# mx-strk/InformationBottleneckDecodingLDPC

Measured on AMD Instinct MI355X. Metric: decoded codewords/sec + achieved HBM GB/s, DVB-S2 N=64800 i_max=50, higher is better.
Workload: dtype u4

## Files before the change

### informationbottleneckdecodingldpc_amd/csrc/ib_kernels.hip

```cpp
#include <algorithm>
#include <type_traits>

#include "common.h"

namespace ibl {


typedef __attribute__((address_space(3))) const uint8_t lds8_t;
__device__ __forceinline__ uint32_t lu(uint32_t x, uint32_t c) {
  asm("" : "+v"(x));
  return *(lds8_t*)(size_t)(x + c);
}
__device__ __forceinline__ uint32_t luc(uint32_t t, uint32_t q, uint32_t c) {
  uint32_t x;
  static_assert(kRowSh == 12, "luc's shift is the row shift of the table layout");
  asm("v_lshl_or_b32 %0, %1, 12, %2" : "=v"(x) : "v"(t), "v"(q));
  return *(lds8_t*)(size_t)(x + c);
}
typedef __attribute__((address_space(3))) const uint64_t lds64_t;
__device__ __forceinline__ uint64_t colf(uint32_t m, uint32_t cb) {
  uint32_t x;
  asm("v_lshl_or_b32 %0, %1, 8, %2" : "=v"(x) : "v"(m), "v"(cb));
  return *(lds64_t*)(size_t)x;
}
__device__ __forceinline__ uint32_t csel(uint64_t col, uint32_t sh) {
  uint64_t r;
  asm("v_lshrrev_b64 %0, %1, %2" : "=v"(r) : "v"(sh), "v"(col));
  return (uint32_t)r;
}
__device__ __forceinline__ uint32_t lds_base(const uint8_t* p) { return (uint32_t)(size_t)(lds8_t*)p; }
__device__ __forceinline__ void lds_at_zero(const uint8_t* lds) {
  if (lds_base(lds) != 0u) __builtin_trap();
}

__device__ __forceinline__ uint32_t qidx(uint32_t m, uint32_t lane4) { return (m << kColSh) | lane4; }

__device__ __forceinline__ uint32_t valid_mask4(int remaining) {
  return remaining >= 4 ? 0xFu : (remaining <= 0 ? 0u : ((1u << remaining) - 1u));
}

__device__ __forceinline__ bool gate_open(const int32_t* gate, int lane) {
  if (!gate) return true;
  return __ballot(gate[lane] != 0) != 0ull;
}

constexpr int kStageR = 4;
#ifndef IBL_STAGE_UNITS
#define IBL_STAGE_UNITS 0
#endif
__device__ __forceinline__ void stage_tables(uint8_t* lds, const uint32_t* img, int nreg) {
  if constexpr (IBL_STAGE_UNITS) {
    uint4* l4 = reinterpret_cast<uint4*>(lds);
    const int n = (int)(lds_of_quads(nreg) / 16), bd = blockDim.x;
    for (int u = threadIdx.x; u < n; u += 4 * bd) {
      uint32_t w[4];
      bool ok[4];
#pragma unroll
      for (int k = 0; k < 4; ++k) {
        const int v = u + k * bd, q = ((v >> 12) << 1) | ((v >> 3) & 1);
        ok[k] = v < n && q < nreg;
        w[k] = ok[k] ? img[q * 256 + ((v >> 4) & 255)] : 0u;
      }
#pragma unroll
      for (int k = 0; k < 4; ++k)
        if (ok[k]) l4[u + k * bd] = make_uint4(w[k], w[k], w[k], w[k]);
    }
    return;
  }
  const int nraw = nreg * 256, lane = threadIdx.x & 63;
  const int wv = threadIdx.x >> 6, nwv = blockDim.x >> 6, nchunk = (nraw + 63) >> 6;
  for (int c0 = 0; c0 < nchunk; c0 += kStageR * nwv) {
    uint32_t v[kStageR];
#pragma unroll
    for (int k = 0; k < kStageR; ++k) {
      const int r = (c0 + wv + k * nwv) * 64 + lane;
      v[k] = r < nraw ? img[r] : 0u;
    }
#pragma unroll
    for (int k = 0; k < kStageR; ++k) {
      const int c = c0 + wv + k * nwv;
      if (c >= nchunk) break;
#pragma unroll
      for (int p = 0; p < 8; ++p) {
        const int src = 8 * p + (lane >> 3), r = c * 64 + src;
        const uint32_t w = __shfl(v[k], src, 64);
        if (r < nraw)
          *reinterpret_cast<uint4*>(lds + quad_off(r >> 8) + (uint32_t)(r & 255) * 256u + 16u * (uint32_t)(lane & 7)) =
              make_uint4(w, w, w, w);
      }
    }
  }
}

__device__ __forceinline__ void stage_cols(uint8_t* dst, const uint32_t* cimg, int ncs) {
  uint32_t* l32 = reinterpret_cast<uint32_t*>(dst);
  const int n = ncs * 1024;
  for (int i = threadIdx.x; i < n; i += blockDim.x) l32[i] = cimg[((i >> 10) << 5) | (((i >> 6) & 15) << 1) | (i & 1)];
}

__device__ __forceinline__ uint32_t nib(uint32_t w, int k) { return __builtin_amdgcn_ubfe(w, 4 * k, 4); }
__device__ __forceinline__ uint32_t colq(uint32_t w, int k, uint32_t lane4) {
  static_assert(kColSh == 8, "colq places the column in byte 1");
  const uint32_t src = (k & 1) ? ((w >> 4) & 0x0F0F0F0Fu) : (w & 0x0F0F0F0Fu);
  return __builtin_amdgcn_perm(src, lane4, 0x03020000u | ((4u + (uint32_t)(k >> 1)) << 8));
}

__device__ __forceinline__ uint32_t valid_nib8(int remaining) {
  return remaining >= 8 ? 0xFFFFFFFFu : (remaining <= 0 ? 0u : ((1u << (4 * remaining)) - 1u));
}

template <int W> struct RowVec;
template <> struct RowVec<1> { typedef uint32_t T; };
template <> struct RowVec<2> { typedef uint2 T; };
template <> struct RowVec<4> { typedef uint4 T; };

#ifndef IBL_NT_CN
#define IBL_NT_CN 1
#endif
#ifndef IBL_NT
#define IBL_NT 1
#endif
typedef uint32_t u32x2_t __attribute__((ext_vector_type(2)));
typedef uint32_t u32x4_t __attribute__((ext_vector_type(4)));
template <int W> struct RowNV;
template <> struct RowNV<1> { typedef uint32_t T; };
template <> struct RowNV<2> { typedef u32x2_t T; };
template <> struct RowNV<4> { typedef u32x4_t T; };

template <int W, bool NT = false>
__device__ __forceinline__ void load_row(const uint8_t* p, uint32_t (&r)[W]) {
  if constexpr (NT) {
    using T = typename RowNV<W>::T;
    const T v = __builtin_nontemporal_load(reinterpret_cast<const T*>(p));
    if constexpr (W == 1) {
      r[0] = v;
    } else {
#pragma unroll
      for (int i = 0; i < W; ++i) r[i] = v[i];
    }
  } else {
    const auto v = *reinterpret_cast<const typename RowVec<W>::T*>(p);
    if constexpr (W == 1) {
      r[0] = v;
    } else if constexpr (W == 2) {
      r[0] = v.x; r[1] = v.y;
    } else {
      r[0] = v.x; r[1] = v.y; r[2] = v.z; r[3] = v.w;
    }
  }
}

template <int W, bool NT = false>
__device__ __forceinline__ void store_row(uint8_t* p, const uint32_t (&r)[W]) {
  if constexpr (NT) {
    using T = typename RowNV<W>::T;
    T v;
    if constexpr (W == 1) {
      v = r[0];
    } else {
#pragma unroll
      for (int i = 0; i < W; ++i) v[i] = r[i];
    }
    __builtin_nontemporal_store(v, reinterpret_cast<T*>(p));
  } else if constexpr (W == 1) {
    *reinterpret_cast<uint32_t*>(p) = r[0];
  } else if constexpr (W == 2) {
    *reinterpret_cast<uint2*>(p) = make_uint2(r[0], r[1]);
  } else {
    *reinterpret_cast<uint4*>(p) = make_uint4(r[0], r[1], r[2], r[3]);
  }
}


template <int MAXD>
constexpr int rowW() { return MAXD <= 8 ? kW : 1; }
template <int MAXD>
constexpr int chunkOf() { return 512 * rowW<MAXD>(); }
static_assert(kLightD <= 8, "light item buffers must fit the MAXD=8 bodies");

template <int MAXD, int W_ = rowW<MAXD>()>
struct ItemBuf {
  static constexpr int kMax = MAXD, W = W_;
  uint32_t row[MAXD][W];
  uint32_t tgv;
  uint32_t chw[W];
  int d, st, node;
  uint32_t off;
  int cwb;
  int fc, fv0, fv1, fd0, fd1;
};

struct PhaseItems {
  int first, pos0, nch;
};

template <class Buf, bool VN, bool GATHER, int FOLD = 0>
__device__ __forceinline__ void fetch_item(const IbFastArgs& a, int item, int lane, Buf& b, const PhaseItems& pi) {
  constexpr int W = Buf::W, MAXD = Buf::kMax;
  const int rel = item - pi.first;
  const int q = __builtin_amdgcn_readfirstlane(rel / pi.nch);
  const int chunk = __builtin_amdgcn_readfirstlane(rel - q * pi.nch);
  const int pos = pi.pos0 + q;
  const int node = sload(a.info, 4 * pos);
  b.node = node;
  b.st = sload(a.info, 4 * pos + 1);
  b.d = sload(a.info, 4 * pos + 2);
  if constexpr (FOLD != 0) {
    const int32_t* rec = a.fold + (size_t)kIbFoldRec * node;
    b.fc = sload(rec, 0);
    b.fv0 = sload(rec, 1);
    b.fv1 = sload(rec, 2);
    b.fd0 = sload(rec, 3);
    b.fd1 = sload(rec, 4);
  }
  b.off = (uint32_t)(chunk * (256 * W) + lane * 4 * W);
  b.cwb = chunk * (512 * W) + lane * 8 * W;
#pragma unroll
  for (int j = 0; j < MAXD; ++j) {
    const int e = b.st + min(j, b.d - 1);
    const uint8_t* row = GATHER ? a.ch8 + (size_t)sload(a.gather, e) * a.ldb : a.in + (size_t)e * a.ldb;
    load_row<W, VN ? (bool)IBL_NT : ((bool)IBL_NT_CN && !GATHER)>(row + b.off, b.row[j]);
  }
  if (VN) {
    load_row<W, IBL_NT>(a.ch8 + (size_t)node * a.ldb + b.off, b.chw);
  } else {
#pragma unroll
    for (int i = 0; i < W; ++i) b.chw[i] = 0;
  }
  b.tgv = (uint32_t)a.tgt[b.st + min(lane, b.d - 1)];
}

template <bool VN, class Buf>
__device__ __forceinline__ void settle(const Buf& b) {
  constexpr int W = Buf::W;
#pragma unroll
  for (int j = 0; j < Buf::kMax; ++j)
#pragma unroll
    for (int i = 0; i < W; ++i) asm volatile("" ::"v"(b.row[j][i]));
  if constexpr (VN) {
#pragma unroll
    for (int i = 0; i < W; ++i) asm volatile("" ::"v"(b.chw[i]));
  }
  asm volatile("" ::"v"(b.tgv));
}

__device__ __forceinline__ uint32_t pack4n(const uint32_t (&t)[4], int g) {
  return (t[0] | (t[1] << 4) | (t[2] << 8) | (t[3] << 12)) << (16 * g);
}

#ifndef IBL_SCHED_FILE
#define IBL_SCHED_FILE "ib_sched.inc"
#endif
#include IBL_SCHED_FILE

template <int D, int NCW = 8>
__device__ __forceinline__ void cn_word(uint32_t lane4, const uint32_t (&in)[D], uint32_t fbase,
                                        const uint32_t (&cb)[4], uint32_t (&outw)[D]) {
#pragma unroll 1
  for (int k0 = 0; k0 < NCW; k0 += cn_sched_s(D)) cn_group<D>(lane4, in, fbase, cb, outw, k0);
}

template <int D, int FC>
__device__ __forceinline__ void cn_word_fold(uint32_t lane4, const uint32_t (&in)[D], uint32_t fbase,
                                             const uint32_t (&cb)[4], uint32_t lane4c, uint32_t ch0, uint32_t ch1,
                                             uint32_t (&outw)[D]) {
#pragma unroll 1
  for (int k0 = 0; k0 < 8; k0 += cn_sched_s(D)) cn_group_fold<D, FC>(lane4, in, fbase, cb, lane4c, ch0, ch1, outw, k0);
}
__device__ __forceinline__ uint32_t fold_word(uint32_t w, uint32_t ch, uint32_t lane4c) {
  uint32_t r = 0;
#pragma unroll
  for (int g = 0; g < 2; ++g) {
    uint32_t t[4];
#pragma unroll
    for (int s = 0; s < 4; ++s) t[s] = luc(nib(w, 4 * g + s), colq(ch, 4 * g + s, lane4c), 0u);
    r |= pack4n(t, g);
  }
  return r;
}

__device__ __forceinline__ void col_bases(const int8_t (&cc)[4], uint32_t lane8c, uint32_t (&cb)[4]) {
#pragma unroll
  for (int i = 0; i < 4; ++i) cb[i] = lane8c + ((uint32_t)cc[i] << 12);
}

template <int D, bool GATHER, class Buf, int FC = 0, bool KEEP = false>
__device__ __forceinline__ void cn_compute(const IbFastArgs& a, uint32_t lane4, uint32_t lane8c, const Buf& b,
                                           int fslot, bool do_par, bool& unsat, uint8_t* fout = nullptr) {
  constexpr int W = Buf::W;
  uint32_t outw[D][W], trow[D], cb[4];
  uint32_t chf[2][W] = {};
  if constexpr (FC != 0 && !GATHER) {
    if constexpr ((FC & 1) != 0) load_row<W>(a.ch8 + (size_t)b.fv0 * (uint32_t)a.ldb + b.off, chf[0]);
    if constexpr ((FC & 2) != 0) load_row<W>(a.ch8 + (size_t)b.fv1 * (uint32_t)a.ldb + b.off, chf[1]);
  }
  col_bases(a.ccol[D], lane8c, cb);
#pragma unroll
  for (int w = 0; w < D; ++w) trow[w] = __builtin_amdgcn_readlane(b.tgv, w);
  const uint32_t fbase = slot_off(fslot);
  if (do_par) {
    const uint32_t bias = (uint32_t)(8 - a.half) * 0x11111111u;
    uint32_t any = 0;
#pragma unroll
    for (int i = 0; i < W; ++i) {
      uint32_t x = (D & 1) ? 0x88888888u : 0u;
#pragma unroll
      for (int j = 0; j < D; ++j) x ^= b.row[j][i] + bias;
      any |= x & 0x88888888u & valid_nib8(a.B - b.cwb - 8 * i);
    }
    if (__ballot(any != 0) != 0ull) unsat = true;
  }
#pragma unroll
  for (int i = 0; i < W; ++i) {
    uint32_t in[D], o[D];
#pragma unroll
    for (int j = 0; j < D; ++j) {
      in[j] = b.row[j][i];
      o[j] = 0;
    }
    if constexpr (D == 2) {
      if (a.match) {
#pragma unroll
        for (int g = 0; g < 2; ++g) {
          uint32_t t0[4], t1[4];
#pragma unroll
          for (int s = 0; s < 4; ++s) {
            t0[s] = lu((nib(in[1], 4 * g + s) << kRowSh) + lane4, fbase);
            t1[s] = lu((nib(in[0], 4 * g + s) << kRowSh) + lane4, fbase);
          }
          o[0] |= pack4n(t0, g);
          o[1] |= pack4n(t1, g);
        }
      } else {
        o[0] = in[1];
        o[1] = in[0];
      }
    } else if constexpr (FC != 0 && !KEEP) {
      const uint32_t c0 = GATHER ? in[D - 2] : chf[0][i], c1 = GATHER ? in[D - 1] : chf[1][i];
      cn_word_fold<D, FC>(lane4, in, fbase, cb, lane4 + slot_off(a.fold_slot), c0, c1, o);
    } else {
      cn_word<D>(lane4, in, fbase, cb, o);
    }
#pragma unroll
    for (int w = 0; w < D; ++w) outw[w][i] = o[w];
  }
  if constexpr (FC == 0 || KEEP) {
#pragma unroll
    for (int w = 0; w < D; ++w) store_row<W, (bool)IBL_NT_CN>(a.out + (size_t)trow[w] * (uint32_t)a.ldb + b.off, outw[w]);
  }
  if constexpr (FC != 0 && KEEP) {
    const uint32_t lane4c = lane4 + slot_off(a.fold_slot);
#pragma unroll
    for (int fa = 0; fa < 2; ++fa) {
      if (!((FC >> fa) & 1)) continue;
      uint32_t fw[W];
#pragma unroll
      for (int i = 0; i < W; ++i) fw[i] = fold_word(outw[D - 2 + fa][i], GATHER ? b.row[D - 2 + fa][i] : chf[fa][i], lane4c);
      store_row<W, (bool)IBL_NT_CN>(fout + (size_t)(uint32_t)(fa ? b.fd1 : b.fd0) * (uint32_t)a.ldb + b.off, fw);
    }
  } else if constexpr (FC != 0) {
#pragma unroll
    for (int w = 0; w < D - 2; ++w) store_row<W, (bool)IBL_NT_CN>(a.out + (size_t)trow[w] * (uint32_t)a.ldb + b.off, outw[w]);
    if constexpr ((FC & 1) != 0) {
      store_row<W, (bool)IBL_NT_CN>(fout + (size_t)(uint32_t)b.fd0 * (uint32_t)a.ldb + b.off, outw[D - 2]);
    } else {
      store_row<W, (bool)IBL_NT_CN>(a.out + (size_t)trow[D - 2] * (uint32_t)a.ldb + b.off, outw[D - 2]);
    }
    if constexpr ((FC & 2) != 0) {
      store_row<W, (bool)IBL_NT_CN>(fout + (size_t)(uint32_t)b.fd1 * (uint32_t)a.ldb + b.off, outw[D - 1]);
    } else {
      store_row<W, (bool)IBL_NT_CN>(a.out + (size_t)trow[D - 1] * (uint32_t)a.ldb + b.off, outw[D - 1]);
    }
  }
}

template <int D, bool GATHER, bool KEEP, class Buf>
__device__ __forceinline__ void cn_compute_fold(const IbFastArgs& a, uint32_t lane4, uint32_t lane8c, const Buf& b,
                                                int fslot, bool do_par, bool& unsat) {
  if constexpr (D >= 3 && D <= 8) {
    uint8_t* fout = a.fout;
    asm volatile("" : "+s"(fout));
    switch (b.fc) {
      case 1: cn_compute<D, GATHER, Buf, 1, KEEP>(a, lane4, lane8c, b, fslot, do_par, unsat, fout); return;
      case 2: cn_compute<D, GATHER, Buf, 2, KEEP>(a, lane4, lane8c, b, fslot, do_par, unsat, fout); return;
      case 3: cn_compute<D, GATHER, Buf, 3, KEEP>(a, lane4, lane8c, b, fslot, do_par, unsat, fout); return;
      default: break;
    }
  }
  cn_compute<D, GATHER>(a, lane4, lane8c, b, fslot, do_par, unsat);
}

template <int D, int NCW = 8>
__device__ __forceinline__ void vn_word(uint32_t lane4, const uint32_t (&in)[D], uint32_t chw,
                                        uint32_t fbase, const uint32_t (&cb)[4], uint32_t (&outw)[D]) {
#pragma unroll 1
  for (int k0 = 0; k0 < NCW; k0 += vn_sched_s(D)) vn_group<D>(lane4, in, chw, fbase, cb, outw, k0);
}

template <int D, class Buf>
__device__ __forceinline__ void vn_compute(const IbFastArgs& a, uint32_t lane4, uint32_t lane8c, const Buf& b,
                                           int fslot) {
  constexpr int W = Buf::W;
  uint32_t outw[D][W], trow[D], cb[4];
  col_bases(a.ccol[D], lane8c, cb);
#pragma unroll
  for (int w = 0; w < D; ++w) trow[w] = __builtin_amdgcn_readlane(b.tgv, w);
  const uint32_t fbase = slot_off(fslot);
#pragma unroll
  for (int i = 0; i < W; ++i) {
    if constexpr (D == 1) {
      outw[0][i] = b.chw[i];
    } else {
      uint32_t in[D], o[D];
#pragma unroll
      for (int j = 0; j < D; ++j) {
        in[j] = b.row[j][i];
        o[j] = 0;
      }
      vn_word<D>(lane4, in, b.chw[i], fbase, cb, o);
#pragma unroll
      for (int w = 0; w < D; ++w) outw[w][i] = o[w];
    }
  }
#pragma unroll
  for (int w = 0; w < D; ++w) store_row<W, IBL_NT>(a.out + (size_t)trow[w] * (uint32_t)a.ldb + b.off, outw[w]);
}

__device__ __forceinline__ void store4(void* out, int dtype, size_t row_off, int cw0, int B, bool aligned,
                                       uint32_t packed) {
  if (dtype == kU8) {
    uint8_t* p = reinterpret_cast<uint8_t*>(out) + row_off + cw0;
    if (aligned && cw0 + 4 <= B) {
      *reinterpret_cast<uint32_t*>(p) = packed;
    } else {
#pragma unroll
      for (int s = 0; s < 4; ++s)
        if (cw0 + s < B) p[s] = (uint8_t)(packed >> (8 * s));
    }
  } else {
    int32_t* p = reinterpret_cast<int32_t*>(out) + row_off + cw0;
    if (aligned && cw0 + 4 <= B) {
      int4 v = make_int4(packed & 0xff, (packed >> 8) & 0xff, (packed >> 16) & 0xff, packed >> 24);
      *reinterpret_cast<int4*>(p) = v;
    } else {
#pragma unroll
      for (int s = 0; s < 4; ++s)
        if (cw0 + s < B) p[s] = (int32_t)((packed >> (8 * s)) & 0xff);
    }
  }
}

template <int D>
__device__ __forceinline__ void dec_item(const IbDecArgs& a, uint32_t lane4, int node,
                                         int st, uint32_t off, int cwb) {
  uint32_t inw[D];
#pragma unroll
  for (int j = 0; j < D; ++j) inw[j] = *reinterpret_cast<const uint32_t*>(a.vin + (size_t)(st + j) * a.ldb + off);
  const uint32_t cw = *reinterpret_cast<const uint32_t*>(a.ch8 + (size_t)node * a.ldb + off);
#pragma unroll
  for (int g = 0; g < 2; ++g) {
    if (cwb + 4 * g >= a.B) break;
    uint32_t packed = 0;
#pragma unroll
    for (int s = 0; s < 4; ++s) {
      const int k = 4 * g + s;
      uint32_t Q = lu((nib(cw, k) << kRowSh) + qidx(nib(inw[0], k), lane4), 0);
#pragma unroll
      for (int l = 1; l < D; ++l) Q = luc(Q, qidx(nib(inw[l], k), lane4), slot_off(l));
      packed |= Q << (8 * s);
    }
    store4(a.out, a.out_dtype, (size_t)node * a.B, cwb + 4 * g, a.B, a.aligned != 0, packed);
  }
}

#define IBL_DEG_CASES(X) X(2) X(3) X(4) X(5) X(6) X(7) X(8) X(9) X(10) X(11) X(12) X(13) X(14) X(15) X(16)
#define IBL_DEG_CASES8(X) X(2) X(3) X(4) X(5) X(6) X(7) X(8)

__device__ __forceinline__ int* lds_counters(const uint8_t* lds, const IbFastArgs& a) {
  return reinterpret_cast<int*>(const_cast<uint8_t*>(lds) + lds_of_quads(a.nt) + (size_t)a.ncs * kColImg);
// ... 205 lines not shown
#define IBL_WPE8C IBL_WPE8
#endif
template <int MAXD, bool GATHER, int FOLD = 0>
__global__ __launch_bounds__(MAXD <= 8 ? IBL_LB8C : IBL_LB16, MAXD <= 8 ? IBL_WPE8C : 1) void ib_cn_fast(IbFastArgs a) {
  static_assert(FOLD == 0 || MAXD <= 8, "the max-degree-16 bodies do not fold");
  extern __shared__ __attribute__((aligned(16))) uint8_t lds[];
  if (!gate_open(a.gate, threadIdx.x & 63)) return;
  lds_at_zero(lds);
  stage_pass(lds, a);
  __syncthreads();
  ib_pass<MAXD, false, GATHER, FOLD>(a, lds);
}

template <int MAXD>
__global__ __launch_bounds__(MAXD <= 8 ? IBL_LB8 : IBL_LB16, MAXD <= 8 ? IBL_WPE8 : 1) void ib_vn_fast(IbFastArgs a) {
  extern __shared__ __attribute__((aligned(16))) uint8_t lds[];
  if (!gate_open(a.gate, threadIdx.x & 63)) return;
  lds_at_zero(lds);
  stage_pass(lds, a);
  __syncthreads();
  ib_pass<MAXD, true, false>(a, lds);
}

__global__ __launch_bounds__(1024) void ib_dec_fast(IbDecArgs a) {
  extern __shared__ __attribute__((aligned(16))) uint8_t lds[];
  const int lane = threadIdx.x & 63;
  const int L = __builtin_amdgcn_readfirstlane(*a.iters);
  lds_at_zero(lds);
  stage_tables(lds, a.img + (size_t)L * a.nt * 256, a.nt);
  __syncthreads();
  const uint32_t lane4 = (uint32_t)(lane & 31) << 2;
  const int wpb = blockDim.x >> 6;
  const int gw = blockIdx.x * wpb + (threadIdx.x >> 6), nw = gridDim.x * wpb;
  const int nitems = a.n_nodes * a.nchunks;
  for (int item = gw; item < nitems; item += nw) {
    const int node = __builtin_amdgcn_readfirstlane(item / a.nchunks);
    const int chunk = __builtin_amdgcn_readfirstlane(item - node * a.nchunks);
    const int d = a.deg[node], st = a.start[node];
    const uint32_t off = (uint32_t)(chunk * (kChunkDec / 2) + lane * 4);
    const int cwb = chunk * kChunkDec + lane * 8;
    if (cwb >= a.B) continue;
    switch (d) {
      case 1: dec_item<1>(a, lane4, node, st, off, cwb); break;
#define X(D) case D: dec_item<D>(a, lane4, node, st, off, cwb); break;
      IBL_DEG_CASES(X)
#undef X
      default: break;
    }
  }
}

template <int D, bool GATHER>
__device__ __forceinline__ void cn_small_item(const IbFastArgs& a, uint32_t lane4, int st, int c, bool do_par,
                                              bool& unsat) {
  uint32_t in[D], o[D];
  int tg[D];
  const uint32_t off = 4u * (uint32_t)c;
#pragma unroll
  for (int j = 0; j < D; ++j) {
    const int e = st + j;
    const uint8_t* row = GATHER ? a.ch8 + (size_t)a.gather[e] * a.ldb : a.in + (size_t)e * a.ldb;
    in[j] = *reinterpret_cast<const uint32_t*>(row + off);
    tg[j] = a.tgt[e];
    o[j] = 0;
  }
  if (do_par) {
    const uint32_t bias = (uint32_t)(8 - a.half) * 0x11111111u;
    uint32_t x = (D & 1) ? 0x88888888u : 0u;
#pragma unroll
    for (int j = 0; j < D; ++j) x ^= in[j] + bias;
    if (x & 0x88888888u & valid_nib8(a.B - 8 * c)) unsat = true;
  }
  const uint32_t fbase = slot_off(a.fslot[D]);
  if constexpr (D == 2) {
    if (a.match) {
#pragma unroll
      for (int g = 0; g < 2; ++g) {
        uint32_t t0[4], t1[4];
#pragma unroll
        for (int s = 0; s < 4; ++s) {
          t0[s] = lu((nib(in[1], 4 * g + s) << kRowSh) + lane4, fbase);
          t1[s] = lu((nib(in[0], 4 * g + s) << kRowSh) + lane4, fbase);
        }
        o[0] |= pack4n(t0, g);
        o[1] |= pack4n(t1, g);
      }
    } else {
      o[0] = in[1];
      o[1] = in[0];
    }
  } else {
    const uint32_t cb[4] = {0, 0, 0, 0};
    if (a.B - 8 * c <= 4) cn_word<D, 4>(lane4, in, fbase, cb, o);
    else cn_word<D>(lane4, in, fbase, cb, o);
  }
#pragma unroll
  for (int w = 0; w < D; ++w) *reinterpret_cast<uint32_t*>(a.out + (size_t)tg[w] * a.ldb + off) = o[w];
}

template <int D>
__device__ __forceinline__ void vn_small_item(const IbFastArgs& a, uint32_t lane4, int node, int st, int c) {
  uint32_t in[D], o[D];
  int tg[D];
  const uint32_t off = 4u * (uint32_t)c;
#pragma unroll
  for (int j = 0; j < D; ++j) {
    in[j] = *reinterpret_cast<const uint32_t*>(a.in + (size_t)(st + j) * a.ldb + off);
    tg[j] = a.tgt[st + j];
    o[j] = 0;
  }
  const uint32_t chw = *reinterpret_cast<const uint32_t*>(a.ch8 + (size_t)node * a.ldb + off);
  if constexpr (D == 1) {
    o[0] = chw;
  } else {
    const uint32_t cb[4] = {0, 0, 0, 0};
    if (a.B - 8 * c <= 4) vn_word<D, 4>(lane4, in, chw, slot_off(a.fslot[D]), cb, o);
    else vn_word<D>(lane4, in, chw, slot_off(a.fslot[D]), cb, o);
  }
#pragma unroll
  for (int w = 0; w < D; ++w) *reinterpret_cast<uint32_t*>(a.out + (size_t)tg[w] * a.ldb + off) = o[w];
}

#ifndef IBL_SMALL_CONTIG
#define IBL_SMALL_CONTIG 1
#endif
template <bool NODE, class Args, class Body>
__device__ __forceinline__ void small_items(const Args& a, int lane, Body&& body) {
  const int wpb = blockDim.x >> 6;
  const int gw = __builtin_amdgcn_readfirstlane(blockIdx.x * wpb + (threadIdx.x >> 6));
  const int nw = gridDim.x * wpb, nitems = a.n_tasks * a.nwords;
  for (int item = gw; item < nitems; item += nw) {
    const int t = __builtin_amdgcn_readfirstlane(item / a.nwords);
    const int c = __builtin_amdgcn_readfirstlane(item - t * a.nwords);
    const int p0 = sload(a.task, 4 * t), cnt = sload(a.task, 4 * t + 1), d = sload(a.task, 4 * t + 2);
    const int st1 = IBL_SMALL_CONTIG ? sload(a.task, 4 * t + 3) : 0;
    if (lane < cnt) {
      int node = 0, st;
      if (st1 != 0) {
        st = st1 - 1 + lane * d;
        if constexpr (NODE) node = sload(a.info, 4 * p0) + lane;
      } else {
        st = a.info[4 * (p0 + lane) + 1];
        if constexpr (NODE) node = a.info[4 * (p0 + lane)];
      }
      body(node, st, c, d);
    }
  }
}

template <int MAXD, bool GATHER>
__global__ __launch_bounds__(kSmallBlock) void ib_cn_small(IbFastArgs a) {
  extern __shared__ __attribute__((aligned(16))) uint8_t lds[];
  const int lane = threadIdx.x & 63;
  if (!gate_open(a.gate, lane)) return;
  lds_at_zero(lds);
  stage_tables(lds, a.img, a.nt);
  __syncthreads();
  const uint32_t lane4 = (uint32_t)(lane & 31) << 2;
  const bool do_par = !GATHER && a.unsat != nullptr;
  bool unsat = false;
  small_items<false>(a, lane, [&](int, int st, int c, int d) __attribute__((always_inline)) {
    switch (d) {
#define X(D) case D: if constexpr (D <= MAXD) cn_small_item<D, GATHER>(a, lane4, st, c, do_par, unsat); break;
      IBL_DEG_CASES(X)
#undef X
      default: break;
    }
  });
  if (do_par && __ballot(unsat) != 0ull && lane == 0)
    atomicOr(&a.unsat[(blockIdx.x * (blockDim.x >> 6) + (threadIdx.x >> 6)) & (kShards - 1)], 1);
}

template <int MAXD>
__global__ __launch_bounds__(kSmallBlock) void ib_vn_small(IbFastArgs a) {
  extern __shared__ __attribute__((aligned(16))) uint8_t lds[];
  const int lane = threadIdx.x & 63;
  if (!gate_open(a.gate, lane)) return;
  lds_at_zero(lds);
  stage_tables(lds, a.img, a.nt);
  __syncthreads();
  const uint32_t lane4 = (uint32_t)(lane & 31) << 2;
  small_items<true>(a, lane, [&](int node, int st, int c, int d) __attribute__((always_inline)) {
    switch (d) {
      case 1: vn_small_item<1>(a, lane4, node, st, c); break;
#define X(D) case D: if constexpr (D <= MAXD) vn_small_item<D>(a, lane4, node, st, c); break;
      IBL_DEG_CASES(X)
#undef X
      default: break;
    }
  });
}

__global__ __launch_bounds__(kSmallBlock) void ib_dec_small(IbDecArgs a) {
  extern __shared__ __attribute__((aligned(16))) uint8_t lds[];
  const int lane = threadIdx.x & 63;
  const int L = __builtin_amdgcn_readfirstlane(*a.iters);
  lds_at_zero(lds);
  stage_tables(lds, a.img + (size_t)L * a.nt * 256, a.nt);
  __syncthreads();
  const uint32_t lane4 = (uint32_t)(lane & 31) << 2;
  small_items<true>(a, lane, [&](int node, int st, int c, int d) __attribute__((always_inline)) {
    const uint32_t off = 4u * (uint32_t)c;
    switch (d) {
      case 1: dec_item<1>(a, lane4, node, st, off, 8 * c); break;
#define X(D) case D: dec_item<D>(a, lane4, node, st, off, 8 * c); break;
      IBL_DEG_CASES(X)
#undef X
      default: break;
    }
  });
}

#ifndef IBL_FUSED_UNROLL
#define IBL_FUSED_UNROLL 1
#endif
template <int D, int NCW>
__device__ __forceinline__ void fused_cn_word(uint32_t lane4, const uint32_t (&in)[D], uint32_t fbase,
                                              const uint32_t (&cb)[4], uint32_t (&o)[D]) {
  if constexpr (IBL_FUSED_UNROLL && D <= 6) {
#pragma unroll
    for (int k0 = 0; k0 < NCW; k0 += cn_sched_s(D)) cn_group<D>(lane4, in, fbase, cb, o, k0);
  } else {
    cn_word<D, NCW>(lane4, in, fbase, cb, o);
  }
}
template <int D, int NCW>
__device__ __forceinline__ void fused_vn_word(uint32_t lane4, const uint32_t (&in)[D], uint32_t chw, uint32_t fbase,
                                              const uint32_t (&cb)[4], uint32_t (&o)[D]) {
  if constexpr (IBL_FUSED_UNROLL && D <= 4) {
#pragma unroll
    for (int k0 = 0; k0 < NCW; k0 += vn_sched_s(D)) vn_group<D>(lane4, in, chw, fbase, cb, o, k0);
  } else {
    vn_word<D, NCW>(lane4, in, chw, fbase, cb, o);
  }
}

template <int D, int NCW>
__device__ __forceinline__ void fused_cn_dword(uint32_t* msg, int first, int cnt, int lane, uint32_t lane4,
                                               const IbFusedArgs& a, bool do_par, uint32_t vmask, bool& unsat) {
  uint32_t in[D], o[D];
#pragma unroll
  for (int j = 0; j < D; ++j) {
    in[j] = msg[first + j * cnt + lane];
    o[j] = 0;
  }
  if (do_par) {
    const uint32_t bias = (uint32_t)(8 - a.half) * 0x11111111u;
    uint32_t x = (D & 1) ? 0x88888888u : 0u;
#pragma unroll
    for (int j = 0; j < D; ++j) x ^= in[j] + bias;
    if (x & 0x88888888u & vmask) unsat = true;
  }
  const uint32_t fbase = slot_off(a.cn_fslot[D]);
  if constexpr (D == 2) {
    if (a.match) {
#pragma unroll
      for (int g = 0; g < NCW / 4; ++g) {
        uint32_t t0[4], t1[4];
#pragma unroll
        for (int s = 0; s < 4; ++s) {
          t0[s] = lu((nib(in[1], 4 * g + s) << kRowSh) + lane4, fbase);
          t1[s] = lu((nib(in[0], 4 * g + s) << kRowSh) + lane4, fbase);
        }
        o[0] |= pack4n(t0, g);
        o[1] |= pack4n(t1, g);
      }
    } else {
      o[0] = in[1];
      o[1] = in[0];
    }
  } else {
    const uint32_t cb[4] = {0, 0, 0, 0};
    fused_cn_word<D, NCW>(lane4, in, fbase, cb, o);
  }
#pragma unroll
  for (int j = 0; j < D; ++j) msg[first + j * cnt + lane] = o[j];
}

template <int MAXD>
struct VnTask {
  int pos, cnt, d, sf;
  uint32_t chw;
  int32_t sl[MAXD];
};

template <int MAXD>
__device__ __forceinline__ void fetch_vn_task(const IbFusedArgs& a, const uint32_t* chg, int t, int lane,
                                              VnTask<MAXD>& v, uint32_t csh) {
  if (a.vn_uni) {
    v.pos = 64 * t;
    v.cnt = min(64, a.n_v - v.pos);
    v.d = a.vn_uni;
    v.sf = v.pos * v.d;
  } else {
    v.pos = sload(a.vn_task, 4 * t);
    v.cnt = sload(a.vn_task, 4 * t + 1);
    v.d = sload(a.vn_task, 4 * t + 2);
    v.sf = sload(a.vn_task, 4 * t + 3);
  }
  const int li = min(lane, v.cnt - 1);
  v.chw = chg[v.pos + li] >> csh;
#pragma unroll
  for (int k = 0; k < MAXD; ++k) v.sl[k] = a.vn_slot[v.sf + min(k, v.d - 1) * v.cnt + li];
}

template <int MAXD>
__device__ __forceinline__ void settle_vn(const VnTask<MAXD>& v) {
  asm volatile("" ::"v"(v.chw));
#pragma unroll
  for (int k = 0; k < MAXD; ++k) asm volatile("" ::"v"(v.sl[k]));
}

template <int D, int MAXD, int NCW>
__device__ __forceinline__ void fused_vn_dword(uint32_t* msg, const VnTask<MAXD>& v, uint32_t lane4,
                                               const IbFusedArgs& a) {
  uint32_t in[D], o[D];
#pragma unroll
  for (int k = 0; k < D; ++k) {
    in[k] = msg[v.sl[k]];
    o[k] = 0;
  }
  if constexpr (D == 1) {
    o[0] = v.chw;
  } else {
    const uint32_t cb[4] = {0, 0, 0, 0};
    fused_vn_word<D, NCW>(lane4, in, v.chw, slot_off(a.vn_fslot[D]), cb, o);
  }
#pragma unroll
  for (int k = 0; k < D; ++k) msg[v.sl[k]] = o[k];
}

template <int D, int MAXD, int NCW>
__device__ __forceinline__ void fused_dec_dword(const uint32_t* msg, const VnTask<MAXD>& v, uint32_t lane4,
                                                uint32_t (&res)[2]) {
  uint32_t in[D];
#pragma unroll
  for (int k = 0; k < D; ++k) in[k] = msg[v.sl[k]];
#pragma unroll
  for (int g = 0; g < NCW / 4; ++g) {
    uint32_t packed = 0;
#pragma unroll
    for (int s = 0; s < 4; ++s) {
      const int k = 4 * g + s;
      uint32_t Q = lu((nib(v.chw, k) << kRowSh) + qidx(nib(in[0], k), lane4), 0);
#pragma unroll
      for (int l = 1; l < D; ++l) Q = luc(Q, qidx(nib(in[l], k), lane4), slot_off(l));
      packed |= Q << (8 * s);
    }
// ... 721 lines not shown
```

Before: 195,600.

## Add compile-time unrolled CN/VN group bodies with scheduling fences and lshl_or packing

Replaces the runtime-looped check-node and variable-node table-lookup groups with generated, fully compile-time-unrolled bodies for degrees up to 8. Nibble pairs are pre-merged into row/column bytes, and packing uses v_lshl_or accumulation. sched_barrier fences pin the instruction order between lookup stages. The aim is to cut address arithmetic and loop overhead and keep LDS lookups interleaved. In exchange it adds code size and register pressure, and the fences may block useful compiler scheduling.

```diff
diff --git a/informationbottleneckdecodingldpc_amd/csrc/ib_kernels.hip b/informationbottleneckdecodingldpc_amd/csrc/ib_kernels.hip
--- a/informationbottleneckdecodingldpc_amd/csrc/ib_kernels.hip
+++ b/informationbottleneckdecodingldpc_amd/csrc/ib_kernels.hip
@@ -104,6 +104,55 @@
   const uint32_t src = (k & 1) ? ((w >> 4) & 0x0F0F0F0Fu) : (w & 0x0F0F0F0Fu);
   return __builtin_amdgcn_perm(src, lane4, 0x03020000u | ((4u + (uint32_t)(k >> 1)) << 8));
 }
+
+template <int P>
+__device__ __forceinline__ uint32_t rowcol(uint32_t x, uint32_t y) {
+  if constexpr (P == 0) return ((x << 4) & 0xF0F0F0F0u) | (y & 0x0F0F0F0Fu);
+  else return (x & 0xF0F0F0F0u) | ((y >> 4) & 0x0F0F0F0Fu);
+}
+__device__ __forceinline__ uint32_t colb(uint32_t e, int k, uint32_t lane4) {
+  return __builtin_amdgcn_perm(e, lane4, 0x03020000u | ((4u + (uint32_t)(k >> 1)) << 8));
+}
+template <int K>
+__device__ __forceinline__ uint32_t pk(uint32_t acc, uint32_t t) {
+  static_assert(K >= 0 && K < 8, "nibble of a dword");
+  if constexpr (K == 0) {
+    return t;
+  } else {
+    uint32_t r;
+    asm("v_lshl_or_b32 %0, %1, %2, %3" : "=v"(r) : "v"(t), "n"(4 * K), "v"(acc));
+    return r;
+  }
+}
+
+#ifndef IBL_STEP_FENCE
+#define IBL_STEP_FENCE 1
+#endif
+__device__ __forceinline__ void step_fence() {
+  if constexpr (IBL_STEP_FENCE) __builtin_amdgcn_sched_barrier(0);
+}
+#define IBL_E(e, x, y) const uint32_t e##_0 = rowcol<0>(x, y), e##_1 = rowcol<1>(x, y)
+#define IBL_EP(e, s) ((ST == 2 ? (K0 & 1) : ((s) & 1)) ? e##_1 : e##_0)
+#define IBL_X2(M, ...) M(0, __VA_ARGS__), M(1, __VA_ARGS__)
+#define IBL_X4(M, ...) IBL_X2(M, __VA_ARGS__), M(2, __VA_ARGS__), M(3, __VA_ARGS__)
+#define IBL_Q_(s, q, w, base) q##_##s = colq(w, K0 + ST * s, base)
+#define IBL_QC_(s, q, on, w) q##_##s = (on) ? colq(w, K0 + ST * s, lane4c) : 0u
+#define IBL_LUC_(s, n, p, q, c) n##_##s = luc(p##_##s, q##_##s, c)
+#define IBL_LU1_(s, n, e, base, c) n##_##s = lu(colb(IBL_EP(e, s), K0 + ST * s, base), c)
+#define IBL_LINK_(s, n, on, p, q) n##_##s = (on) ? luc(p##_##s, q##_##s, 0u) : p##_##s
+#define IBL_PK_(s, o, v) o = pk<K0 + ST * s>(o, v##_##s)
+#define IBL_Q2(...) const uint32_t IBL_X2(IBL_Q_, __VA_ARGS__)
+#define IBL_Q4(...) const uint32_t IBL_X4(IBL_Q_, __VA_ARGS__)
+#define IBL_QC2(...) const uint32_t IBL_X2(IBL_QC_, __VA_ARGS__)
+#define IBL_QC4(...) const uint32_t IBL_X4(IBL_QC_, __VA_ARGS__)
+#define IBL_LUC2(...) const uint32_t IBL_X2(IBL_LUC_, __VA_ARGS__)
+#define IBL_LUC4(...) const uint32_t IBL_X4(IBL_LUC_, __VA_ARGS__)
+#define IBL_LU12(...) const uint32_t IBL_X2(IBL_LU1_, __VA_ARGS__)
+#define IBL_LU14(...) const uint32_t IBL_X4(IBL_LU1_, __VA_ARGS__)
+#define IBL_LINK2(...) const uint32_t IBL_X2(IBL_LINK_, __VA_ARGS__)
+#define IBL_LINK4(...) const uint32_t IBL_X4(IBL_LINK_, __VA_ARGS__)
+#define IBL_PK2(...) IBL_X2(IBL_PK_, __VA_ARGS__)
+#define IBL_PK4(...) IBL_X4(IBL_PK_, __VA_ARGS__)
 
 __device__ __forceinline__ uint32_t valid_nib8(int remaining) {
   return remaining >= 8 ? 0xFFFFFFFFu : (remaining <= 0 ? 0u : ((1u << (4 * remaining)) - 1u));
@@ -244,28 +293,79 @@
   asm volatile("" ::"v"(b.tgv));
 }
 
-__device__ __forceinline__ uint32_t pack4n(const uint32_t (&t)[4], int g) {
-  return (t[0] | (t[1] << 4) | (t[2] << 8) | (t[3] << 12)) << (16 * g);
+__device__ __forceinline__ uint32_t pack4n(uint32_t acc, const uint32_t (&t)[4], int g) {
+  return g == 0 ? pk<3>(pk<2>(pk<1>(pk<0>(acc, t[0]), t[1]), t[2]), t[3])
+                : pk<7>(pk<6>(pk<5>(pk<4>(acc, t[0]), t[1]), t[2]), t[3]);
 }
 
 #ifndef IBL_SCHED_FILE
 #define IBL_SCHED_FILE "ib_sched.inc"
 #endif
 #include IBL_SCHED_FILE
-
-template <int D, int NCW = 8>
+#ifndef IBL_WORD_CT
+#define IBL_WORD_CT 1
+#endif
+#ifndef IBL_UNROLLED_FILE
+#define IBL_UNROLLED_FILE "ib_unrolled.inc"
+#endif
+template <int D, int MAXD = 8> constexpr bool kWordCT = IBL_WORD_CT && D <= 8 && MAXD <= 8;
+#if IBL_WORD_CT
+#include IBL_UNROLLED_FILE
+template <int D, int K0, int ST>
+__device__ __forceinline__ void cn_group_ct(uint32_t lane4, const uint32_t (&in)[D], uint32_t fbase, uint32_t (&o)[D]) {
+  cn_group_fold_ct<D, 0, K0, ST>(lane4, in, fbase, 0u, 0u, 0u, o);
+}
+#else
+template <int D, int K0, int ST, class... A> __device__ void cn_group_ct(A...);
+template <int D, int FC, int K0, int ST, class... A> __device__ void cn_group_fold_ct(A...);
+template <int D, int K0, int ST, class... A> __device__ void vn_group_ct(A...);
+#endif
+
+template <int NCW> constexpr int kWordST = NCW == 8 ? 2 : 1;
+template <int S, int NCW>
+__host__ __device__ constexpr int word_k0(int gi) {
+  if (kWordST<NCW> == 1) return gi * S;
+  const int npp = 4 / S;
+  return gi / npp + (gi % npp) * 2 * S;
+}
+template <int D, int GI, int NCW>
+__device__ __forceinline__ void cn_word_ct(uint32_t lane4, const uint32_t (&in)[D], uint32_t fbase,
+                                           uint32_t (&outw)[D]) {
+  constexpr int S = cn_sched_s(D);
+  static_assert(S == 2 || S == 4, "parity groups of 2 or 4 codewords");
+  cn_group_ct<D, word_k0<S, NCW>(GI), kWordST<NCW>>(lane4, in, fbase, outw);
+  if constexpr ((GI + 1) * S < NCW) {
+    __builtin_amdgcn_sched_barrier(0);
+    cn_word_ct<D, GI + 1, NCW>(lane4, in, fbase, outw);
+  }
+}
+template <int D, int NCW = 8, bool CT = false>
 __device__ __forceinline__ void cn_word(uint32_t lane4, const uint32_t (&in)[D], uint32_t fbase,
                                         const uint32_t (&cb)[4], uint32_t (&outw)[D]) {
+  if constexpr (CT) {
+    cn_word_ct<D, 0, NCW>(lane4, in, fbase, outw);
+  } else {
 #pragma unroll 1
-  for (int k0 = 0; k0 < NCW; k0 += cn_sched_s(D)) cn_group<D>(lane4, in, fbase, cb, outw, k0);
-}
-
-template <int D, int FC>
+    for (int k0 = 0; k0 < NCW; k0 += cn_sched_s(D)) cn_group<D>(lane4, in, fbase, cb, outw, k0);
+  }
+}
+
+template <int D, int FC, int GI = 0>
 __device__ __forceinline__ void cn_word_fold(uint32_t lane4, const uint32_t (&in)[D], uint32_t fbase,
                                              const uint32_t (&cb)[4], uint32_t lane4c, uint32_t ch0, uint32_t ch1,
                                              uint32_t (&outw)[D]) {
+  if constexpr (kWordCT<D>) {
+    constexpr int S = cn_sched_s(D);
+    static_assert(S == 2 || S == 4, "parity groups of 2 or 4 codewords");
+    cn_group_fold_ct<D, FC, word_k0<S, 8>(GI), kWordST<8>>(lane4, in, fbase, lane4c, ch0, ch1, outw);
+    if constexpr ((GI + 1) * S < 8) {
+      __builtin_amdgcn_sched_barrier(0);
+      cn_word_fold<D, FC, GI + 1>(lane4, in, fbase, cb, lane4c, ch0, ch1, outw);
+    }
+  } else {
 #pragma unroll 1
-  for (int k0 = 0; k0 < 8; k0 += cn_sched_s(D)) cn_group_fold<D, FC>(lane4, in, fbase, cb, lane4c, ch0, ch1, outw, k0);
+    for (int k0 = 0; k0 < 8; k0 += cn_sched_s(D)) cn_group_fold<D, FC>(lane4, in, fbase, cb, lane4c, ch0, ch1, outw, k0);
+  }
 }
 __device__ __forceinline__ uint32_t fold_word(uint32_t w, uint32_t ch, uint32_t lane4c) {
   uint32_t r = 0;
@@ -274,7 +374,7 @@
     uint32_t t[4];
 #pragma unroll
     for (int s = 0; s < 4; ++s) t[s] = luc(nib(w, 4 * g + s), colq(ch, 4 * g + s, lane4c), 0u);
-    r |= pack4n(t, g);
+    r = pack4n(r, t, g);
   }
   return r;
 }
@@ -313,6 +413,9 @@
 #pragma unroll
   for (int i = 0; i < W; ++i) {
     uint32_t in[D], o[D];
+    if constexpr (kWordCT<D, Buf::kMax>) {
+      if (i) __builtin_amdgcn_sched_barrier(0);
+    }
 #pragma unroll
     for (int j = 0; j < D; ++j) {
       in[j] = b.row[j][i];
@@ -328,8 +431,8 @@
             t0[s] = lu((nib(in[1], 4 * g + s) << kRowSh) + lane4, fbase);
             t1[s] = lu((nib(in[0], 4 * g + s) << kRowSh) + lane4, fbase);
           }
-          o[0] |= pack4n(t0, g);
-          o[1] |= pack4n(t1, g);
+          o[0] = pack4n(o[0], t0, g);
+          o[1] = pack4n(o[1], t1, g);
         }
       } else {
         o[0] = in[1];
@@ -339,7 +442,7 @@
       const uint32_t c0 = GATHER ? in[D - 2] : chf[0][i], c1 = GATHER ? in[D - 1] : chf[1][i];
       cn_word_fold<D, FC>(lane4, in, fbase, cb, lane4 + slot_off(a.fold_slot), c0, c1, o);
     } else {
-      cn_word<D>(lane4, in, fbase, cb, o);
+      cn_word<D, 8, kWordCT<D, Buf::kMax>>(lane4, in, fbase, cb, o);
     }
 #pragma unroll
     for (int w = 0; w < D; ++w) outw[w][i] = o[w];
@@ -390,11 +493,26 @@
   cn_compute<D, GATHER>(a, lane4, lane8c, b, fslot, do_par, unsat);
 }
 
-template <int D, int NCW = 8>
+template <int D, int GI, int NCW>
+__device__ __forceinline__ void vn_word_ct(uint32_t lane4, const uint32_t (&in)[D], uint32_t chw,
+                                           uint32_t fbase, uint32_t (&outw)[D]) {
+  constexpr int S = vn_sched_s(D);
+  static_assert(S == 2 || S == 4, "parity groups of 2 or 4 codewords");
+  vn_group_ct<D, word_k0<S, NCW>(GI), kWordST<NCW>>(lane4, in, fbase, chw, outw);
+  if constexpr ((GI + 1) * S < NCW) {
+    __builtin_amdgcn_sched_barrier(0);
+    vn_word_ct<D, GI + 1, NCW>(lane4, in, chw, fbase, outw);
+  }
+}
+template <int D, int NCW = 8, bool CT = false>
 __device__ __forceinline__ void vn_word(uint32_t lane4, const uint32_t (&in)[D], uint32_t chw,
                                         uint32_t fbase, const uint32_t (&cb)[4], uint32_t (&outw)[D]) {
+  if constexpr (CT) {
+    vn_word_ct<D, 0, NCW>(lane4, in, chw, fbase, outw);
+  } else {
 #pragma unroll 1
-  for (int k0 = 0; k0 < NCW; k0 += vn_sched_s(D)) vn_group<D>(lane4, in, chw, fbase, cb, outw, k0);
+    for (int k0 = 0; k0 < NCW; k0 += vn_sched_s(D)) vn_group<D>(lane4, in, chw, fbase, cb, outw, k0);
+  }
 }
 
 template <int D, class Buf>
@@ -766,8 +884,8 @@
           t0[s] = lu((nib(in[1], 4 * g + s) << kRowSh) + lane4, fbase);
           t1[s] = lu((nib(in[0], 4 * g + s) << kRowSh) + lane4, fbase);
         }
-        o[0] |= pack4n(t0, g);
-        o[1] |= pack4n(t1, g);
+        o[0] = pack4n(o[0], t0, g);
+        o[1] = pack4n(o[1], t1, g);
       }
     } else {
       o[0] = in[1];
@@ -901,7 +1019,9 @@
 template <int D, int NCW>
 __device__ __forceinline__ void fused_cn_word(uint32_t lane4, const uint32_t (&in)[D], uint32_t fbase,
                                               const uint32_t (&cb)[4], uint32_t (&o)[D]) {
-  if constexpr (IBL_FUSED_UNROLL && D <= 6) {
+  if constexpr (IBL_FUSED_UNROLL && IBL_WORD_CT && D <= 6) {
+    cn_word<D, NCW, true>(lane4, in, fbase, cb, o);
+  } else if constexpr (IBL_FUSED_UNROLL && D <= 6) {
 #pragma unroll
     for (int k0 = 0; k0 < NCW; k0 += cn_sched_s(D)) cn_group<D>(lane4, in, fbase, cb, o, k0);
   } else {
@@ -911,7 +1031,9 @@
 template <int D, int NCW>
 __device__ __forceinline__ void fused_vn_word(uint32_t lane4, const uint32_t (&in)[D], uint32_t chw, uint32_t fbase,
                                               const uint32_t (&cb)[4], uint32_t (&o)[D]) {
-  if constexpr (IBL_FUSED_UNROLL && D <= 4) {
+  if constexpr (IBL_FUSED_UNROLL && IBL_WORD_CT && D <= 4) {
+    vn_word<D, NCW, true>(lane4, in, chw, fbase, cb, o);
+  } else if constexpr (IBL_FUSED_UNROLL && D <= 4) {
 #pragma unroll
     for (int k0 = 0; k0 < NCW; k0 += vn_sched_s(D)) vn_group<D>(lane4, in, chw, fbase, cb, o, k0);
   } else {
@@ -946,8 +1068,8 @@
           t0[s] = lu((nib(in[1], 4 * g + s) << kRowSh) + lane4, fbase);
           t1[s] = lu((nib(in[0], 4 * g + s) << kRowSh) + lane4, fbase);
         }
-        o[0] |= pack4n(t0, g);
-        o[1] |= pack4n(t1, g);
+        o[0] = pack4n(o[0], t0, g);
+        o[1] = pack4n(o[1], t1, g);
       }
     } else {
       o[0] = in[1];
diff --git a/informationbottleneckdecodingldpc_amd/csrc/ib_unrolled.inc b/informationbottleneckdecodingldpc_amd/csrc/ib_unrolled.inc
--- /dev/null
+++ b/informationbottleneckdecodingldpc_amd/csrc/ib_unrolled.inc
@@ -0,0 +1,336 @@
+static_assert(cn_sched_s(8) == 4 && vn_sched_s(8) == 2 && cn_ncols(7) == 0 && vn_ncols(8) == 0,
+              "the unrolled bodies were generated for another schedule (IBL_UNROLLED_FILE)");
+template <int D, int FC, int K0, int ST> __device__ __forceinline__ void cn_group_fold_ct(uint32_t lane4, const uint32_t (&in)[D], uint32_t fbase, uint32_t lane4c, uint32_t ch0, uint32_t ch1,
+    uint32_t (&o)[D]) {
+  static_assert(D >= 3 && D <= 8 && K0 >= 0 && (ST == 1 || ST == 2), "unrolled bodies: degrees 3..8");
+  if constexpr (D == 3) {
+    const uint32_t lane4f = lane4 + fbase;
+    IBL_E(E0_1, in[0], in[1]);
+    IBL_E(E0_2, in[0], in[2]);
+    IBL_E(E1_2, in[1], in[2]);
+    IBL_LU14(v_P_0, E0_1, lane4f, 0u);
+    IBL_LU14(v_o0_0, E1_2, lane4f, 0u);
+    step_fence();
+    IBL_QC4(qc1, FC & 2, ch1);
+    IBL_LINK4(f_P, FC & 2, v_P_0, qc1);
+    IBL_LU14(v_c1_0, E0_2, lane4f, 0u);
+    IBL_PK4(o[0], v_o0_0);
+    step_fence();
+    IBL_QC4(qc0, FC & 1, ch0);
+    IBL_LINK4(f_c1, FC & 1, v_c1_0, qc0);
+    IBL_PK4(o[2], f_P);
+    step_fence();
+    IBL_PK4(o[1], f_c1);
+    step_fence();
+  }
+  if constexpr (D == 4) {
+    const uint32_t lane4f = lane4 + fbase;
+    IBL_E(E0_1, in[0], in[1]);
+    IBL_E(E0_2, in[0], in[2]);
+    IBL_E(E1_2, in[1], in[2]);
+    IBL_LU14(v_P_0, E0_1, lane4, 0u);
+    IBL_LU14(v_o0_0, E1_2, lane4, 0u);
+    step_fence();
+    IBL_Q4(q2, in[2], lane4f);
+    IBL_Q4(q3, in[3], lane4f);
+    IBL_LUC4(v_P_1, v_P_0, q2, 0u);
+    IBL_LUC4(v_o0_1, v_o0_0, q3, 0u);
+    step_fence();
+    IBL_QC4(qc1, FC & 2, ch1);
+    IBL_LINK4(f_P, FC & 2, v_P_1, qc1);
+    IBL_LU14(v_c1_0, E0_2, lane4, 0u);
+    IBL_LUC4(v_c2_0, v_P_0, q3, 0u);
+    IBL_PK4(o[0], v_o0_1);
+    step_fence();
+    IBL_QC4(qc0, FC & 1, ch0);
+    IBL_LINK4(f_c2, FC & 1, v_c2_0, qc0);
+    IBL_LUC4(v_c1_1, v_c1_0, q3, 0u);
+    IBL_PK4(o[3], f_P);
+    step_fence();
+    IBL_PK4(o[2], f_c2);
+    IBL_PK4(o[1], v_c1_1);
+    step_fence();
+  }
+  if constexpr (D == 5) {
+    const uint32_t lane4f = lane4 + fbase;
+    IBL_E(E0_1, in[0], in[1]);
+    IBL_E(E0_2, in[0], in[2]);
+    IBL_E(E1_2, in[1], in[2]);
+    IBL_LU14(v_P_0, E0_1, lane4, 0u);
+    IBL_LU14(v_o0_0, E1_2, lane4, 0u);
+    step_fence();
+    IBL_Q4(q2, in[2], lane4);
+    IBL_Q4(q3, in[3], lane4);
+    IBL_LUC4(v_P_1, v_P_0, q2, 1u);
+    IBL_LUC4(v_o0_1, v_o0_0, q3, 1u);
+    step_fence();
+    IBL_Q4(q4, in[4], lane4f);
+    IBL_LUC4(v_P_2, v_P_1, q3, fbase);
+    IBL_LUC4(v_o0_2, v_o0_1, q4, 0u);
+    step_fence();
+    IBL_QC4(qc1, FC & 2, ch1);
+    IBL_LINK4(f_P, FC & 2, v_P_2, qc1);
+    IBL_LU14(v_c1_0, E0_2, lane4, 0u);
+    IBL_LUC4(v_c2_0, v_P_0, q3, 1u);
+    IBL_PK4(o[0], v_o0_2);
+    step_fence();
+    IBL_LUC4(v_c1_1, v_c1_0, q3, 1u);
+    IBL_LUC4(v_c2_1, v_c2_0, q4, 0u);
+    IBL_PK4(o[4], f_P);
+    step_fence();
+    IBL_LUC4(v_c1_2, v_c1_1, q4, 0u);
+    IBL_LUC4(v_c3_0, v_P_1, q4, 0u);
+    IBL_PK4(o[2], v_c2_1);
+    step_fence();
+    IBL_QC4(qc0, FC & 1, ch0);
+    IBL_LINK4(f_c3, FC & 1, v_c3_0, qc0);
+    IBL_PK4(o[1], v_c1_2);
+    step_fence();
+    IBL_PK4(o[3], f_c3);
+    step_fence();
+  }
+  if constexpr (D == 6) {
+    const uint32_t lane4f = lane4 + fbase;
+    IBL_E(E0_1, in[0], in[1]);
+    IBL_E(E0_2, in[0], in[2]);
+    IBL_E(E1_2, in[1], in[2]);
+    IBL_LU14(v_P_0, E0_1, lane4, 0u);
+    IBL_LU14(v_o0_0, E1_2, lane4, 0u);
+    step_fence();
+    IBL_Q4(q2, in[2], lane4);
+    IBL_Q4(q3, in[3], lane4);
+    IBL_LUC4(v_P_1, v_P_0, q2, 1u);
+    IBL_LUC4(v_o0_1, v_o0_0, q3, 1u);
+    step_fence();
+    IBL_Q4(q4, in[4], lane4);
+    IBL_LUC4(v_P_2, v_P_1, q3, 2u);
+    IBL_LUC4(v_o0_2, v_o0_1, q4, 2u);
+    step_fence();
+    IBL_Q4(q5, in[5], lane4f);
+    IBL_LUC4(v_P_3, v_P_2, q4, fbase);
+    IBL_LUC4(v_o0_3, v_o0_2, q5, 0u);
+    step_fence();
+    IBL_QC4(qc1, FC & 2, ch1);
+    IBL_LINK4(f_P, FC & 2, v_P_3, qc1);
+    IBL_LU14(v_c1_0, E0_2, lane4, 0u);
+    IBL_LUC4(v_c2_0, v_P_0, q3, 1u);
+    IBL_PK4(o[0], v_o0_3);
+    step_fence();
+    IBL_LUC4(v_c1_1, v_c1_0, q3, 1u);
+    IBL_LUC4(v_c2_1, v_c2_0, q4, 2u);
+    IBL_PK4(o[5], f_P);
+    step_fence();
+    IBL_LUC4(v_c1_2, v_c1_1, q4, 2u);
+    IBL_LUC4(v_c2_2, v_c2_1, q5, 0u);
+    step_fence();
+    IBL_LUC4(v_c1_3, v_c1_2, q5, 0u);
+    IBL_LUC4(v_c3_0, v_P_1, q4, 2u);
+    IBL_PK4(o[2], v_c2_2);
+    step_fence();
+    IBL_LUC4(v_c3_1, v_c3_0, q5, 0u);
+    IBL_LUC4(v_c4_0, v_P_2, q5, 0u);
+    IBL_PK4(o[1], v_c1_3);
+    step_fence();
+    IBL_QC4(qc0, FC & 1, ch0);
+    IBL_LINK4(f_c4, FC & 1, v_c4_0, qc0);
+    IBL_PK4(o[3], v_c3_1);
+    step_fence();
+    IBL_PK4(o[4], f_c4);
+    step_fence();
+  }
+  if constexpr (D == 7) {
+    const uint32_t lane4f = lane4 + fbase;
+    IBL_E(E0_1, in[0], in[1]);
+    IBL_E(E0_2, in[0], in[2]);
+    IBL_E(E1_2, in[1], in[2]);
+    IBL_LU14(v_P_0, E0_1, lane4, 0u);
+    IBL_LU14(v_o0_0, E1_2, lane4, 0u);
+    step_fence();
+    IBL_Q4(q2, in[2], lane4);
+    IBL_Q4(q3, in[3], lane4);
+    IBL_LUC4(v_P_1, v_P_0, q2, 1u);
+    IBL_LUC4(v_o0_1, v_o0_0, q3, 1u);
+    step_fence();
+    IBL_Q4(q4, in[4], lane4);
+    IBL_LUC4(v_P_2, v_P_1, q3, 2u);
+    IBL_LUC4(v_o0_2, v_o0_1, q4, 2u);
+    step_fence();
+    IBL_Q4(q5, in[5], lane4);
+    IBL_LUC4(v_P_3, v_P_2, q4, 3u);
+    IBL_LUC4(v_o0_3, v_o0_2, q5, 3u);
+    step_fence();
+    IBL_Q4(q6, in[6], lane4f);
+    IBL_LUC4(v_P_4, v_P_3, q5, fbase);
+    IBL_LUC4(v_o0_4, v_o0_3, q6, 0u);
+    step_fence();
+    IBL_QC4(qc1, FC & 2, ch1);
+    IBL_LINK4(f_P, FC & 2, v_P_4, qc1);
+    IBL_LU14(v_c1_0, E0_2, lane4, 0u);
+    IBL_LUC4(v_c2_0, v_P_0, q3, 1u);
+    IBL_PK4(o[0], v_o0_4);
+    step_fence();
+    IBL_LUC4(v_c1_1, v_c1_0, q3, 1u);
+    IBL_LUC4(v_c2_1, v_c2_0, q4, 2u);
+    IBL_PK4(o[6], f_P);
+    step_fence();
+    IBL_LUC4(v_c1_2, v_c1_1, q4, 2u);
+    IBL_LUC4(v_c2_2, v_c2_1, q5, 3u);
+    step_fence();
+    IBL_LUC4(v_c1_3, v_c1_2, q5, 3u);
+    IBL_LUC4(v_c2_3, v_c2_2, q6, 0u);
+    step_fence();
+    IBL_LUC4(v_c1_4, v_c1_3, q6, 0u);
+    IBL_LUC4(v_c3_0, v_P_1, q4, 2u);
+    IBL_PK4(o[2], v_c2_3);
+    step_fence();
+    IBL_LUC4(v_c3_1, v_c3_0, q5, 3u);
+    IBL_LUC4(v_c4_0, v_P_2, q5, 3u);
+    IBL_PK4(o[1], v_c1_4);
+    step_fence();
+    IBL_LUC4(v_c3_2, v_c3_1, q6, 0u);
+    IBL_LUC4(v_c4_1, v_c4_0, q6, 0u);
+    step_fence();
+    IBL_LUC4(v_c5_0, v_P_3, q6, 0u);
+    IBL_PK4(o[3], v_c3_2);
+    IBL_PK4(o[4], v_c4_1);
+    step_fence();
+    IBL_QC4(qc0, FC & 1, ch0);
+    IBL_LINK4(f_c5, FC & 1, v_c5_0, qc0);
+    step_fence();
+    IBL_PK4(o[5], f_c5);
+    step_fence();
+  }
+  if constexpr (D == 8) {
+    const uint32_t lane4f = lane4 + fbase;
+    IBL_E(E0_1, in[0], in[1]);
+    IBL_E(E0_2, in[0], in[2]);
+    IBL_E(E1_2, in[1], in[2]);
+    IBL_LU14(v_P_0, E0_1, lane4, 0u);
+    IBL_LU14(v_o0_0, E1_2, lane4, 0u);
+    step_fence();
+    IBL_Q4(q2, in[2], lane4);
+    IBL_Q4(q3, in[3], lane4);
+    IBL_LUC4(v_P_1, v_P_0, q2, 1u);
+    IBL_LUC4(v_o0_1, v_o0_0, q3, 1u);
+    step_fence();
+    IBL_Q4(q4, in[4], lane4);
+    IBL_LUC4(v_P_2, v_P_1, q3, 2u);
+    IBL_LUC4(v_o0_2, v_o0_1, q4, 2u);
+    step_fence();
+    IBL_Q4(q5, in[5], lane4);
+    IBL_LUC4(v_P_3, v_P_2, q4, 3u);
+    IBL_LUC4(v_o0_3, v_o0_2, q5, 3u);
+    step_fence();
+    IBL_Q4(q6, in[6], lane4);
+    IBL_LUC4(v_P_4, v_P_3, q5, 128u);
+    IBL_LUC4(v_o0_4, v_o0_3, q6, 128u);
+    step_fence();
+    IBL_Q4(q7, in[7], lane4f);
+    IBL_LUC4(v_P_5, v_P_4, q6, fbase);
+    IBL_LUC4(v_o0_5, v_o0_4, q7, 0u);
+    step_fence();
+    IBL_QC4(qc1, FC & 2, ch1);
+    IBL_LINK4(f_P, FC & 2, v_P_5, qc1);
+    IBL_LU14(v_c1_0, E0_2, lane4, 0u);
+    IBL_LUC4(v_c2_0, v_P_0, q3, 1u);
+    IBL_PK4(o[0], v_o0_5);
+    step_fence();
+    IBL_LUC4(v_c1_1, v_c1_0, q3, 1u);
+    IBL_LUC4(v_c2_1, v_c2_0, q4, 2u);
+    IBL_PK4(o[7], f_P);
+    step_fence();
+    IBL_LUC4(v_c1_2, v_c1_1, q4, 2u);
+    IBL_LUC4(v_c2_2, v_c2_1, q5, 3u);
+    step_fence();
+    IBL_LUC4(v_c1_3, v_c1_2, q5, 3u);
+    IBL_LUC4(v_c2_3, v_c2_2, q6, 128u);
+    step_fence();
+    IBL_LUC4(v_c1_4, v_c1_3, q6, 128u);
+    IBL_LUC4(v_c2_4, v_c2_3, q7, 0u);
+    step_fence();
+    IBL_LUC4(v_c1_5, v_c1_4, q7, 0u);
+    IBL_LUC4(v_c3_0, v_P_1, q4, 2u);
+    IBL_PK4(o[2], v_c2_4);
+    step_fence();
+    IBL_LUC4(v_c3_1, v_c3_0, q5, 3u);
+    IBL_LUC4(v_c4_0, v_P_2, q5, 3u);
+    IBL_PK4(o[1], v_c1_5);
+    step_fence();
+    IBL_LUC4(v_c3_2, v_c3_1, q6, 128u);
+    IBL_LUC4(v_c4_1, v_c4_0, q6, 128u);
+    step_fence();
+    IBL_LUC4(v_c3_3, v_c3_2, q7, 0u);
+    IBL_LUC4(v_c4_2, v_c4_1, q7, 0u);
+    step_fence();
+    IBL_LUC4(v_c5_0, v_P_3, q6, 128u);
+    IBL_LUC4(v_c6_0, v_P_4, q7, 0u);
+    IBL_PK4(o[3], v_c3_3);
+    IBL_PK4(o[4], v_c4_2);
+    step_fence();
+    IBL_QC4(qc0, FC & 1, ch0);
+    IBL_LINK4(f_c6, FC & 1, v_c6_0, qc0);
+    IBL_LUC4(v_c5_1, v_c5_0, q7, 0u);
+    step_fence();
+    IBL_PK4(o[6], f_c6);
+    IBL_PK4(o[5], v_c5_1);
+    step_fence();
+  }
+}
+template <int D, int K0, int ST> __device__ __forceinline__ void vn_group_ct(uint32_t lane4, const uint32_t (&in)[D], uint32_t fbase, uint32_t chw,
+    uint32_t (&o)[D]) {
+  static_assert(D >= 2 && D <= 4 && K0 >= 0 && (ST == 1 || ST == 2), "unrolled bodies: degrees 2..4");
+  if constexpr (D == 2) {
+    const uint32_t lane4f = lane4 + fbase;
+    IBL_E(Ec_0, chw, in[0]);
+    IBL_E(Ec_1, chw, in[1]);
+    IBL_LU12(v_Q_0, Ec_0, lane4f, 0u);
+    IBL_LU12(v_o0_0, Ec_1, lane4f, 0u);
+    step_fence();
+    IBL_PK2(o[1], v_Q_0);
+    IBL_PK2(o[0], v_o0_0);
+    step_fence();
+  }
+  if constexpr (D == 3) {
+    const uint32_t lane4f = lane4 + fbase;
+    IBL_E(Ec_0, chw, in[0]);
+    IBL_E(Ec_1, chw, in[1]);
+    IBL_LU12(v_Q_0, Ec_0, lane4, 0u);
+    IBL_LU12(v_o0_0, Ec_1, lane4, 0u);
+    step_fence();
+    IBL_Q2(q1, in[1], lane4f);
+    IBL_Q2(q2, in[2], lane4f);
+    IBL_LUC2(v_Q_1, v_Q_0, q1, 0u);
+    IBL_LUC2(v_o0_1, v_o0_0, q2, 0u);
+    IBL_LUC2(v_c1_0, v_Q_0, q2, 0u);
+    step_fence();
+    IBL_PK2(o[2], v_Q_1);
+    IBL_PK2(o[0], v_o0_1);
+    IBL_PK2(o[1], v_c1_0);
+    step_fence();
+  }
+  if constexpr (D == 4) {
+    const uint32_t lane4f = lane4 + fbase;
+    IBL_E(Ec_0, chw, in[0]);
+    IBL_E(Ec_1, chw, in[1]);
+    IBL_LU12(v_Q_0, Ec_0, lane4, 0u);
+    IBL_LU12(v_o0_0, Ec_1, lane4, 0u);
+    step_fence();
+    IBL_Q2(q1, in[1], lane4);
+    IBL_Q2(q2, in[2], lane4);
+    IBL_LUC2(v_Q_1, v_Q_0, q1, 1u);
+    IBL_LUC2(v_o0_1, v_o0_0, q2, 1u);
+    IBL_LUC2(v_c1_0, v_Q_0, q2, 1u);
+    step_fence();
+    IBL_Q2(q3, in[3], lane4f);
+    IBL_LUC2(v_Q_2, v_Q_1, q2, fbase);
+    IBL_LUC2(v_o0_2, v_o0_1, q3, 0u);
+    IBL_LUC2(v_c1_1, v_c1_0, q3, 0u);
+    IBL_LUC2(v_c2_0, v_Q_1, q3, 0u);
+    step_fence();
+    IBL_PK2(o[3], v_Q_2);
+    IBL_PK2(o[0], v_o0_2);
+    IBL_PK2(o[1], v_c1_1);
+    IBL_PK2(o[2], v_c2_0);
+    step_fence();
+  }
+}
```

Measured after the change: 203,100 (median of 6 runs). 1.04x the previous value.
